# Jamol/kuma

Hardware: AMD Instinct MI355X
Metric: GiB/s device-resident WS frame mask/unmask, 64 KiB frames; % HBM peak (higher is better)
Workload: dtype u8

## Files before the change

### kuma_amd/csrc/kmws_common.hpp

```cpp
#pragma once
#include <hip/hip_runtime.h>
#include <stdint.h>
#include <string.h>

#include "kmws_gpu.h"

namespace kmws {

typedef uint32_t u32x4 __attribute__((ext_vector_type(4)));

constexpr int kBlock = 256;

struct WsHead {
    uint32_t status;
    uint32_t pad[3];
};
constexpr uint32_t kStatusBadDesc = 1u;
constexpr uint32_t kStatusBadHeader = 2u;
constexpr uint32_t kStatusLookbackTimeout = 4u;

__host__ __device__ __forceinline__ uint64_t splitmix64(uint64_t x)
{
    uint64_t z = x + 0x9E3779B97F4A7C15ull;
    z = (z ^ (z >> 30)) * 0xBF58476D1CE4E5B9ull;
    z = (z ^ (z >> 27)) * 0x94D049BB133111EBull;
    return z ^ (z >> 31);
}

__device__ __forceinline__ uint32_t rot_key(uint32_t key, uint64_t frame_off)
{
    return __builtin_rotateleft32(key, (uint32_t)(frame_off & 3u) * 8u);
}

__device__ __forceinline__ uint32_t dword_byte_mask(int lo, int hi, int d)
{
    int a = lo - 4 * d, b = hi - 4 * d;
    a = a < 0 ? 0 : a;
    b = b > 4 ? 4 : b;
    if (b <= a) return 0u;
    uint32_t hm = b >= 4 ? 0xFFFFFFFFu : ((1u << (8 * b)) - 1u);
    uint32_t lm = (1u << (8 * a)) - 1u;
    return hm & ~lm;
}

__device__ __forceinline__ uint64_t low_bytes64(int k)
{
    return k >= 8 ? ~0ull : ((1ull << (8 * k)) - 1ull);
}
__device__ __forceinline__ u32x4 word_byte_range(int lo, int hi)
{
    const int l0 = lo < 8 ? lo : 8, h0 = hi < 8 ? hi : 8;
    const int l1 = lo > 8 ? lo - 8 : 0, h1 = hi > 8 ? hi - 8 : 0;
    const uint64_t a = low_bytes64(h0) & ~low_bytes64(l0);
    const uint64_t b = low_bytes64(h1) & ~low_bytes64(l1);
    return u32x4{(uint32_t)a, (uint32_t)(a >> 32), (uint32_t)b, (uint32_t)(b >> 32)};
}

inline kmws_status hip_status(hipError_t e)
{
    return e == hipSuccess ? KMWS_OK : KMWS_ERR_FAILED;
}

kmws_status launch_zero(void* p, uint32_t bytes, hipStream_t s);

constexpr uint32_t kPieceWords = 4 * kBlock;
struct PieceRec {
    uint32_t frame;
    uint32_t piece;
};
inline uint64_t piece_count(uint64_t off, uint32_t len)
{
    if (len == 0) return 0;
    const uint64_t words = ((off + len + 15) >> 4) - (off >> 4);
    return (words + kPieceWords - 1) / kPieceWords;
}
kmws_status launch_unmask_pieces(uint8_t* base, const kmws_desc* descs, const PieceRec* pieces, uint32_t np,
                                 hipStream_t s);

int resolve_device(int device);
void note_device_batch(uint64_t bytes, hipStream_t stream);
bool device_batch_running(int device);

constexpr int kResMaxDescs = KMWS_RESIDENT_MAX_PAYLOADS;
constexpr uint64_t kResMaxBytes = KMWS_RESIDENT_MAX_BYTES;
constexpr uint64_t kResMaxBytesAsync = kResMaxBytes;
struct ResidentJob {
    int device = -1;
    int slot = -1;
    uint64_t seq = 0;
};
kmws_status resident_post(int device, const kmws_desc* descs, const uint8_t* dev_base, size_t n,
                          const kmws_desc* descs2, const uint8_t* dev_base2, size_t n2, ResidentJob* job,
                          uint64_t max_bytes = kResMaxBytes);
int resident_test(const ResidentJob& job);
kmws_status resident_wait(const ResidentJob& job);
kmws_status resident_unmask(int device, const kmws_desc* descs, const uint8_t* dev_base, size_t n,
                            const kmws_desc* descs2, const uint8_t* dev_base2, size_t n2);

}
```

### kuma_amd/csrc/kmws_unmask.hip

```cpp
#include "kmws_bench.h"
#include "kmws_common.hpp"
#include "kmws_frame_parse.hpp"

namespace kmws {

constexpr int kBufNT = 2;
constexpr int kBufferRsrcWord3 = 0x00020000;

__device__ __forceinline__ __amdgpu_buffer_rsrc_t tile_rsrc(uint8_t* base, uint64_t lo, uint64_t hi)
{
    return __builtin_amdgcn_make_buffer_rsrc(base + lo, (short)0, (int)((hi - lo + 15) & ~15ull), kBufferRsrcWord3);
}

template <bool NT>
__device__ __forceinline__ void store_word(const u32x4& val, __amdgpu_buffer_rsrc_t rs, uint32_t off)
{
    __builtin_amdgcn_raw_buffer_store_b128(val, rs, (int)off, 0, NT ? kBufNT : 0);
}

template <int V>
struct UnmaskCfg {
    static constexpr int kWords = kBlock * V;
    static constexpr uint64_t kTile = (uint64_t)kWords * 16u;
    static constexpr int kCap = kBlock;
};

__global__ void __launch_bounds__(kBlock) tile_map_kernel(const kmws_desc* __restrict__ d, uint32_t n,
                                                          uint64_t span, uint32_t tile_shift,
                                                          uint32_t* __restrict__ map,
                                                          WsHead* __restrict__ head)
{
    const uint32_t f = blockIdx.x * kBlock + threadIdx.x;
    if (f >= n) return;
    const kmws_desc df = d[f];
    const uint64_t next = (f + 1 < n) ? d[f + 1].off : span;
    if (df.off > span || df.off + (uint64_t)df.len > next) {
        atomicOr(&head->status, kStatusBadDesc);
        return;
    }
    const uint64_t start = f == 0 ? 0 : df.off;
    const uint64_t T = 1ull << tile_shift;
    const uint64_t b0 = (start + T - 1) >> tile_shift;
    const uint64_t b1 = (next + T - 1) >> tile_shift;
    for (uint64_t b = b0; b < b1; ++b) map[b] = f;
    if (f == n - 1) map[b1] = f;
}

__global__ void __launch_bounds__(kBlock) unpack_plan_kernel(const uint8_t* __restrict__ wire, uint64_t span,
                                                             const uint64_t* __restrict__ hdr_off, uint32_t n,
                                                             int mode, kmws_desc* __restrict__ out_desc,
                                                             uint16_t* __restrict__ out_flags,
                                                             uint8_t* __restrict__ out_err, uint32_t tile_shift,
                                                             uint32_t* __restrict__ map, WsHead* __restrict__ head)
{
    const uint32_t f = blockIdx.x * kBlock + threadIdx.x;
    if (f >= n) return;
    unpack_one(wire, span, hdr_off, n, f, mode, out_desc, out_flags, out_err, head);
    const uint64_t h = hdr_off[f];
    const uint64_t next = f + 1 < n ? hdr_off[f + 1] : span;
    if (h > next || next > span) {
        atomicOr(&head->status, kStatusBadDesc);
        return;
    }
    const uint64_t start = f == 0 ? 0 : h;
    const uint64_t T = 1ull << tile_shift;
    const uint64_t b0 = (start + T - 1) >> tile_shift;
    const uint64_t b1 = (next + T - 1) >> tile_shift;
    for (uint64_t b = b0; b < b1; ++b) map[b] = f;
    if (f == n - 1) map[b1] = f;
}

template <int V, bool FULL>
__device__ __forceinline__ void load_tile(const uint8_t* __restrict__ base, uint64_t tile_lo, uint64_t tile_hi,
                                          u32x4 (&v)[V])
{
    const int tid = threadIdx.x;
#pragma unroll
    for (int i = 0; i < V; ++i) {
        const uint64_t a = tile_lo + 16u * (uint64_t)(tid + kBlock * i);
        if (FULL || a < tile_hi) v[i] = __builtin_nontemporal_load(reinterpret_cast<const u32x4*>(base + a));
        else v[i] = u32x4{0, 0, 0, 0};
    }
}

template <int V, bool FULL, bool TWO = false, bool NT = true>
__device__ __forceinline__ void finish_tile(uint8_t* __restrict__ base, uint64_t tile_lo, uint64_t tile_hi,
                                            const kmws_desc* __restrict__ d, uint32_t n,
                                            const uint32_t* __restrict__ map, uint32_t tile, bool ok,
                                            const u32x4 (&v)[V], uint64_t* s_off, uint64_t* s_end, uint32_t* s_key,
                                            const u32x4* pre = nullptr)
{
    using Cfg = UnmaskCfg<V>;
    const int tid = threadIdx.x;
    const __amdgpu_buffer_rsrc_t rs = tile_rsrc(base, tile_lo, tile_hi);
    uint32_t f = map[tile];
    const uint32_t flast = map[tile + 1];

    const kmws_desc d0 = d[f < n ? f : 0];
    if (FULL && f < n && d0.off <= tile_lo && d0.off + d0.len >= tile_hi) {
        const uint32_t r = rot_key(d0.key, d0.off);
#pragma unroll
        for (int i = 0; i < V; ++i) {
            const uint64_t a = tile_lo + 16u * (uint64_t)(tid + kBlock * i);
            if (ok) store_word<NT>(v[i] ^ r, rs, (uint32_t)(a - tile_lo));
        }
        return;
    }

    if (TWO && FULL && flast <= f + 1 && f < n) {
        const kmws_desc d1 = flast > f && flast < n ? d[flast] : kmws_desc{~0ull, 0u, 0u};
        const uint32_t r0 = rot_key(d0.key, d0.off), r1 = rot_key(d1.key, d1.off);
        constexpr uint32_t T = (uint32_t)Cfg::kTile;
        auto rel = [&](uint64_t x) -> uint32_t {
            return x <= tile_lo ? 0u : (x - tile_lo >= T ? T : (uint32_t)(x - tile_lo));
        };
        const uint32_t s0 = rel(d0.off), t0 = rel(d0.off + d0.len);
        const uint32_t s1 = rel(d1.off), t1 = d1.len ? rel(d1.off + d1.len) : s1;
        u32x4 m[V];
#pragma unroll
        for (int i = 0; i < V; ++i) {
            const uint32_t x = 16u * (uint32_t)(tid + kBlock * i);
            u32x4 mm = u32x4{0, 0, 0, 0};
            if (s0 <= x && t0 >= x + 16) {
                mm = u32x4{r0, r0, r0, r0};
            } else if (s1 <= x && t1 >= x + 16) {
                mm = u32x4{r1, r1, r1, r1};
            } else {
                auto cl = [&](uint32_t y) -> int { return y <= x ? 0 : (y - x >= 16u ? 16 : (int)(y - x)); };
                mm = (word_byte_range(cl(s0), cl(t0)) & r0) | (word_byte_range(cl(s1), cl(t1)) & r1);
            }
            m[i] = mm;
        }
        __builtin_amdgcn_sched_barrier(0);
#pragma unroll
        for (int i = 0; i < V; ++i) {
            const uint64_t a = tile_lo + 16u * (uint64_t)(tid + kBlock * i);
            if (ok && (m[i].x | m[i].y | m[i].z | m[i].w) != 0u)
                store_word<NT>(v[i] ^ m[i], rs, (uint32_t)(a - tile_lo));
        }
        return;
    }

    u32x4 m[V];
#pragma unroll
    for (int i = 0; i < V; ++i) m[i] = u32x4{0, 0, 0, 0};
    auto round = [&](bool have, const u32x4& x) -> int {
        int valid = 0;
        if (have) {
            const uint64_t off = (uint64_t)x.x | ((uint64_t)x.y << 32);
            if (off < tile_hi) {
                valid = 1;
                s_off[tid] = off;
                s_end[tid] = off + x.z;
                s_key[tid] = x.w;
            }
        }
        const int cnt = __syncthreads_count(valid);
#pragma unroll
        for (int i = 0; i < V; ++i) {
            const uint64_t a = tile_lo + 16u * (uint64_t)(tid + kBlock * i);
            int lo = 0, hi = cnt;
            while (lo < hi) {
                const int mid = (lo + hi) >> 1;
                if (s_end[mid] <= a) lo = mid + 1; else hi = mid;
            }
            for (int j = lo; j < cnt; ++j) {
                const uint64_t o = s_off[j];
                if (o >= a + 16) break;
                const uint64_t e = s_end[j];
                const uint32_t r = rot_key(s_key[j], o);
                if (o <= a && e >= a + 16) {
                    m[i] |= u32x4{r, r, r, r};
                } else {
                    const int blo = o > a ? (int)(o - a) : 0;
                    const int bhi = e < a + 16 ? (int)(e - a) : 16;
                    m[i].x |= r & dword_byte_mask(blo, bhi, 0);
                    m[i].y |= r & dword_byte_mask(blo, bhi, 1);
                    m[i].z |= r & dword_byte_mask(blo, bhi, 2);
                    m[i].w |= r & dword_byte_mask(blo, bhi, 3);
                }
            }
        }
        __syncthreads();
        return cnt;
    };
    auto have_f = [&]() { return f + (uint32_t)tid < n && f + (uint32_t)tid <= flast; };
    auto load_f = [&]() { return have_f() ? *reinterpret_cast<const u32x4*>(d + f + tid) : u32x4{0, 0, 0, 0}; };
    int cnt = pre ? round(have_f(), *pre) : round(have_f(), load_f());
    while (cnt == Cfg::kCap) {
        f += Cfg::kCap;
        cnt = round(have_f(), load_f());
    }
#pragma unroll
    for (int i = 0; i < V; ++i) {
        const uint64_t a = tile_lo + 16u * (uint64_t)(tid + kBlock * i);
        const u32x4 mm = m[i];
        if (ok && (FULL || a < tile_hi) && (mm.x | mm.y | mm.z | mm.w) != 0u)
            store_word<NT>(v[i] ^ mm, rs, (uint32_t)(a - tile_lo));
    }
}

template <int V>
__global__ void __launch_bounds__(kBlock) unmask_tail_kernel(uint8_t* __restrict__ base, uint64_t span,
                                                             const kmws_desc* __restrict__ d, uint32_t n,
                                                             const uint32_t* __restrict__ map,
                                                             const WsHead* __restrict__ head, uint32_t tile)
{
    using Cfg = UnmaskCfg<V>;
    __shared__ uint64_t s_off[Cfg::kCap];
    __shared__ uint64_t s_end[Cfg::kCap];
    __shared__ uint32_t s_key[Cfg::kCap];
    const uint64_t tile_lo = (uint64_t)tile * Cfg::kTile;
    u32x4 v[V];
    load_tile<V, false>(base, tile_lo, span, v);
    __builtin_amdgcn_sched_barrier(0);
    finish_tile<V, false>(base, tile_lo, span, d, n, map, tile, (head->status & kStatusBadDesc) == 0, v, s_off, s_end, s_key);
}

template <int V, bool TWO = false, bool NT = true>
__global__ void __launch_bounds__(kBlock) unmask_split_kernel(uint8_t* __restrict__ base,
                                                              const kmws_desc* __restrict__ d, uint32_t n,
                                                              const uint32_t* __restrict__ map,
                                                              const WsHead* __restrict__ head, uint32_t nfull,
                                                              uint32_t k, uint32_t c, uint32_t b0, uint32_t w)
{
    using Cfg = UnmaskCfg<V>;
    __shared__ uint64_t s_off[Cfg::kCap];
    __shared__ uint64_t s_end[Cfg::kCap];
    __shared__ uint32_t s_key[Cfg::kCap];
    const uint32_t b = b0 + blockIdx.x;
    uint32_t tile = b;
    if (c == 0) {
        const uint32_t q = nfull / k;
        if (b < q * k) tile = (b % k) * q + b / k;
    } else if (w <= 1) {
        const uint64_t run = (uint64_t)k * c;
        if (b < nfull / run * run) {
            const uint32_t x = b % k, i = b / k;
            tile = (i / c) * (uint32_t)run + x * c + i % c;
        }
    } else {
        const uint32_t kg = k / w;
        const uint64_t run = (uint64_t)kg * c;
        const uint64_t per = (uint64_t)nfull / w / run * run;
        if (b < per * w) {
            const uint32_t x = b % k, i = b / k;
            const uint32_t g = x % w, xi = x / w;
            tile = (uint32_t)(g * per) + (i / c) * (uint32_t)run + xi * c + i % c;
        }
    }
    const uint64_t lo = (uint64_t)tile * Cfg::kTile;
    u32x4 v[V];
    if constexpr (!TWO) {
        const uint32_t f = map[tile], fl = map[tile + 1];
        const uint32_t fi = f + threadIdx.x;
        u32x4 pre = u32x4{0, 0, 0, 0};
        if (fi < n && fi <= fl) pre = *reinterpret_cast<const u32x4*>(d + fi);
        load_tile<V, true>(base, lo, lo + Cfg::kTile, v);
        __builtin_amdgcn_sched_barrier(0);
        finish_tile<V, true, TWO, NT>(base, lo, lo + Cfg::kTile, d, n, map, tile, (head->status & kStatusBadDesc) == 0, v, s_off, s_end,
                                      s_key, &pre);
        return;
    }
    load_tile<V, true>(base, lo, lo + Cfg::kTile, v);
    __builtin_amdgcn_sched_barrier(0);
    finish_tile<V, true, TWO, NT>(base, lo, lo + Cfg::kTile, d, n, map, tile, (head->status & kStatusBadDesc) == 0, v, s_off, s_end,
                                  s_key);
}

__global__ void __launch_bounds__(kBlock) unmask_pieces_kernel(uint8_t* __restrict__ base,
                                                               const kmws_desc* __restrict__ d,
                                                               const PieceRec* __restrict__ pieces)
{
    constexpr int V = kPieceWords / kBlock;
    const PieceRec pr = pieces[blockIdx.x];
    const kmws_desc x = d[pr.frame];
    const uint64_t end = x.off + x.len;
    const uint64_t w0 = (x.off >> 4) + (uint64_t)pr.piece * kPieceWords;
    const uint64_t wh = (end + 15) >> 4;
    const uint64_t w1 = wh < w0 + kPieceWords ? wh : w0 + kPieceWords;
    const uint32_t r = rot_key(x.key, x.off);
    u32x4 v[V];
#pragma unroll
    for (int i = 0; i < V; ++i) {
        const uint64_t w = w0 + threadIdx.x + (uint64_t)kBlock * i;
        v[i] = w < w1 ? *reinterpret_cast<const u32x4*>(base + 16 * w) : u32x4{0, 0, 0, 0};
    }
#pragma unroll
    for (int i = 0; i < V; ++i) {
        const uint64_t w = w0 + threadIdx.x + (uint64_t)kBlock * i;
        if (w >= w1) continue;
        const uint64_t a = 16 * w;
        if (a >= x.off && a + 16 <= end) {
            *reinterpret_cast<u32x4*>(base + a) = v[i] ^ r;
        } else {
            const uint64_t lo = a > x.off ? a : x.off, hi = a + 16 < end ? a + 16 : end;
            for (uint64_t q = lo; q < hi; ++q) {
                const uint32_t b = (uint32_t)(q - a);
                const uint32_t dw = (b & 8u) ? ((b & 4u) ? v[i].w : v[i].z) : ((b & 4u) ? v[i].y : v[i].x);
                base[q] = (uint8_t)((dw ^ r) >> (8 * (b & 3u)));
            }
        }
    }
}

__global__ void __launch_bounds__(kBlock) fill_synthetic_kernel(uint8_t* __restrict__ base, uint64_t bytes,
                                                                uint64_t seed)
{
    const uint64_t nw = bytes >> 4;
    const uint64_t stride = (uint64_t)gridDim.x * kBlock;
    for (uint64_t w = (uint64_t)blockIdx.x * kBlock + threadIdx.x; w < nw; w += stride) {
        const uint64_t a = splitmix64(seed + 2 * w), b = splitmix64(seed + 2 * w + 1);
        *reinterpret_cast<u32x4*>(base + 16 * w) =
            u32x4{(uint32_t)a, (uint32_t)(a >> 32), (uint32_t)b, (uint32_t)(b >> 32)};
    }
    if (blockIdx.x == 0 && threadIdx.x < (bytes & 15)) {
        const uint64_t i = (nw << 4) + threadIdx.x;
        base[i] = (uint8_t)(splitmix64(seed + (i >> 3)) >> (8 * (i & 7)));
    }
}

__global__ void __launch_bounds__(kBlock) uniform_descs_kernel(kmws_desc* __restrict__ d, uint32_t n,
                                                               uint64_t stride, uint32_t len, uint64_t key_seed)
{
    const uint32_t i = blockIdx.x * kBlock + threadIdx.x;
    if (i >= n) return;
    kmws_desc x;
    x.off = (uint64_t)i * stride;
    x.len = len;
    x.key = (uint32_t)splitmix64(key_seed + i);
    d[i] = x;
}

constexpr int kCheckBytes = 4096;

__global__ void __launch_bounds__(kBlock) check_unmasked_kernel(const uint8_t* __restrict__ base, uint64_t bytes,
                                                                uint64_t seed, const kmws_desc* __restrict__ d,
                                                                uint32_t n, unsigned long long* mismatches)
{
    __shared__ uint32_t s_first;
    const uint64_t nblk = (bytes + kCheckBytes - 1) / kCheckBytes;
    unsigned long long bad = 0;
    for (uint64_t blk = blockIdx.x; blk < nblk; blk += gridDim.x) {
    const uint64_t blk_lo = blk * kCheckBytes;
    __syncthreads();
    if (threadIdx.x == 0) {
        uint32_t lo = 0, hi = n;
        while (lo < hi) {
            const uint32_t mid = (lo + hi) >> 1;
            if (d[mid].off + d[mid].len <= blk_lo) lo = mid + 1; else hi = mid;
        }
        s_first = lo;
    }
    __syncthreads();
    uint32_t f = s_first;
    const uint64_t p0 = blk_lo + 16u * threadIdx.x;
    for (int k = 0; k < 16; ++k) {
        const uint64_t p = p0 + k;
        if (p >= bytes) break;
        while (f < n && d[f].off + d[f].len <= p) ++f;
        uint8_t expect = (uint8_t)(splitmix64(seed + (p >> 3)) >> (8 * (p & 7)));
        if (f < n && d[f].off <= p) {
            const uint32_t key = d[f].key;
            expect ^= (uint8_t)(key >> (8 * ((p - d[f].off) & 3)));
        }
        bad += base[p] != expect;
    }
    }
    if (bad) atomicAdd(mismatches, bad);
}

constexpr int kUnmaskV = 4;
using ProdCfg = UnmaskCfg<kUnmaskV>;

constexpr unsigned kUnmaskBlocksPerCu = 2;
constexpr uint32_t kUnmaskStaticLds = ProdCfg::kCap * (8 + 8 + 4);

static unsigned unmask_lds_pad_device()
{
    static thread_local int dev_cached = -1;
    static thread_local unsigned pad = 0;
    int dev = 0;
    if (hipGetDevice(&dev) != hipSuccess) return 0;
    if (dev != dev_cached) {
        int lds = 0;
        pad = 0;
        if (
            hipDeviceGetAttribute(&lds, hipDeviceAttributeMaxSharedMemoryPerMultiprocessor, dev) == hipSuccess &&
            lds > 0) {
            const unsigned per_block = (unsigned)lds / (kUnmaskBlocksPerCu + 1) + 1;
            pad = per_block > kUnmaskStaticLds ? per_block - kUnmaskStaticLds : 0u;
        }
        dev_cached = dev;
    }
    return pad;
}

static unsigned unmask_lds_pad(uint64_t span, uint32_t n)
{
    return n && span / n >= ProdCfg::kTile ? unmask_lds_pad_device() : 0u;
}

static uint32_t ilog2_u64(uint64_t x)
{
    uint32_t r = 0;
    while ((1ull << r) < x) ++r;
    return r;
}

static kmws_status check_ws(uint64_t span, size_t ws_bytes, uint64_t* ntiles_out)
{
    const uint64_t ntiles = (span + ProdCfg::kTile - 1) / ProdCfg::kTile;
    if (ntiles > 0x7FFFFFFFull) return KMWS_ERR_INVALID_PARAM;
    if (ws_bytes < sizeof(WsHead) + (ntiles + 1) * sizeof(uint32_t)) return KMWS_ERR_BUFFER_TOO_SMALL;
    *ntiles_out = ntiles;
    return KMWS_OK;
}

static kmws_status launch_plan(uint64_t span, const kmws_desc* descs, uint32_t n, void* workspace, size_t ws_bytes,
                               hipStream_t s)
{
    uint64_t ntiles = 0;
    kmws_status st = check_ws(span, ws_bytes, &ntiles);
    if (st != KMWS_OK) return st;
    WsHead* head = static_cast<WsHead*>(workspace);
    if (launch_zero(head, sizeof(WsHead), s) != KMWS_OK) return KMWS_ERR_FAILED;
    if (n == 0 || span == 0) return KMWS_OK;
    hipLaunchKernelGGL(tile_map_kernel, dim3((n + kBlock - 1) / kBlock), dim3(kBlock), 0, s, descs, n, span,
                       ilog2_u64(ProdCfg::kTile), reinterpret_cast<uint32_t*>(head + 1), head);
    return hip_status(hipGetLastError());
}

struct Split {
    uint32_t k, c, w;
};
constexpr uint32_t kKindMask = 0xFFu;
constexpr uint32_t kSchedTemporal = KMWS_SCHED_TEMPORAL_STORES;
constexpr uint32_t kSchedNT = KMWS_SCHED_NT_STORES;
static uint32_t default_schedule(uint64_t span, uint32_t n)
{
    return n && span / n >= ProdCfg::kTile ? KMWS_SCHED_SPLIT4 : KMWS_SCHED_GROUPED_RUNS;
}

static bool split_of(uint32_t kind, Split* sp)
{
    switch (kind) {
    case KMWS_SCHED_GROUPED_RUNS: *sp = {8u, 16u, 2u}; return true;
    case KMWS_SCHED_IN_ORDER: *sp = {1u, 0u, 1u}; return true;
    case KMWS_SCHED_SPLIT2: *sp = {2u, 0u, 1u}; return true;
    case KMWS_SCHED_SPLIT8: *sp = {8u, 0u, 1u}; return true;
    case KMWS_SCHED_XCD_RUNS: *sp = {8u, 16u, 1u}; return true;
    case KMWS_SCHED_SPLIT4: *sp = {4u, 0u, 1u}; return true;
    default: return false;
    }
}

static bool valid_schedule(uint32_t code)
{
    Split sp;
    const uint32_t store = code & (kSchedTemporal | kSchedNT);
    return split_of(code & kKindMask, &sp) && store != (kSchedTemporal | kSchedNT) &&
           (code & ~(kKindMask | kSchedTemporal | kSchedNT)) == 0;
}

static bool temporal_stores(uint32_t code) { return (code & kSchedTemporal) != 0; }

static kmws_status launch_apply(uint32_t code, uint8_t* base, uint64_t span, const kmws_desc* descs, uint32_t n,
                                const void* workspace, size_t ws_bytes, hipStream_t s)
{
    Split sp;
    if (!valid_schedule(code) || !split_of(code & kKindMask, &sp)) return KMWS_ERR_INVALID_PARAM;
    uint64_t ntiles = 0;
    kmws_status st = check_ws(span, ws_bytes, &ntiles);
    if (st != KMWS_OK) return st;
    if (n == 0 || span == 0) return KMWS_OK;
    const WsHead* head = static_cast<const WsHead*>(workspace);
    const uint32_t* map = reinterpret_cast<const uint32_t*>(head + 1);
    const uint64_t nfull = span / ProdCfg::kTile;
    const bool temporal = temporal_stores(code);
    constexpr uint64_t kMaxBlocks = (1ull << 32) / kBlock / 2;
    const unsigned lds_pad = unmask_lds_pad(span, n);
    for (uint64_t b0 = 0; b0 < nfull; b0 += kMaxBlocks) {
        const dim3 grid((uint32_t)(nfull - b0 < kMaxBlocks ? nfull - b0 : kMaxBlocks));
        const uint32_t nf = (uint32_t)nfull, bb = (uint32_t)b0;
        if (lds_pad && !temporal)
            hipLaunchKernelGGL((unmask_split_kernel<kUnmaskV, true, true>), grid, dim3(kBlock), lds_pad, s, base, descs,
                               n, map, head, nf, sp.k, sp.c, bb, sp.w);
        else if (lds_pad)
            hipLaunchKernelGGL((unmask_split_kernel<kUnmaskV, true, false>), grid, dim3(kBlock), lds_pad, s, base,
                               descs, n, map, head, nf, sp.k, sp.c, bb, sp.w);
        else if (!temporal)
            hipLaunchKernelGGL((unmask_split_kernel<kUnmaskV, false, true>), grid, dim3(kBlock), 0, s, base, descs, n,
                               map, head, nf, sp.k, sp.c, bb, sp.w);
        else
            hipLaunchKernelGGL((unmask_split_kernel<kUnmaskV, false, false>), grid, dim3(kBlock), 0, s, base, descs,
                               n, map, head, nf, sp.k, sp.c, bb, sp.w);
    }
    if (ntiles > nfull)
        hipLaunchKernelGGL(unmask_tail_kernel<kUnmaskV>, dim3(1), dim3(kBlock), 0, s, base, span, descs, n, map, head,
                           (uint32_t)nfull);
    return hip_status(hipGetLastError());
}

static bool bad_args(const uint8_t* base, const kmws_desc* descs, uint32_t n, const void* ws)
{
    return !ws || (n && (!base || !descs)) || (reinterpret_cast<uintptr_t>(base) & 15u);
}

__global__ void __launch_bounds__(64) zero_kernel(uint64_t* __restrict__ p, uint32_t words)
{
    for (uint32_t i = threadIdx.x; i < words; i += 64) p[i] = 0;
}

kmws_status launch_zero(void* p, uint32_t bytes, hipStream_t s)
{
    if (!p || (bytes & 7u) || bytes > 4096) return KMWS_ERR_INVALID_PARAM;
    hipLaunchKernelGGL(zero_kernel, dim3(1), dim3(64), 0, s, static_cast<uint64_t*>(p), bytes / 8);
    return hip_status(hipGetLastError());
}

kmws_status launch_unmask_pieces(uint8_t* base, const kmws_desc* descs, const PieceRec* pieces, uint32_t np,
                                 hipStream_t s)
{
    if (np == 0) return KMWS_OK;
    if (!base || !descs || !pieces) return KMWS_ERR_INVALID_PARAM;
    hipLaunchKernelGGL(unmask_pieces_kernel, dim3(np), dim3(kBlock), 0, s, base, descs, pieces);
    return hip_status(hipGetLastError());
}
}

using namespace kmws;

extern "C" {

size_t kmws_unmask_workspace_size(uint64_t span)
{
    const uint64_t ntiles = (span + ProdCfg::kTile - 1) / ProdCfg::kTile;
    return sizeof(WsHead) + (size_t)(ntiles + 1) * sizeof(uint32_t);
}

kmws_status kmws_unmask_batch(uint8_t* base, uint64_t span, const kmws_desc* descs, uint32_t n,
                              void* workspace, size_t workspace_bytes, void* stream)
{
    if (bad_args(base, descs, n, workspace)) return KMWS_ERR_INVALID_PARAM;
    kmws_status st = launch_plan(span, descs, n, workspace, workspace_bytes, static_cast<hipStream_t>(stream));
    if (st != KMWS_OK) return st;
    return kmws_unmask_apply(base, span, descs, n, workspace, workspace_bytes, stream);
}

kmws_status kmws_unmask_plan(uint64_t span, const kmws_desc* descs, uint32_t n, void* workspace,
                             size_t workspace_bytes, void* stream)
{
    if (!workspace || (n && !descs)) return KMWS_ERR_INVALID_PARAM;
    return launch_plan(span, descs, n, workspace, workspace_bytes, static_cast<hipStream_t>(stream));
}

kmws_status kmws_unmask_apply(uint8_t* base, uint64_t span, const kmws_desc* descs, uint32_t n,
                              const void* workspace, size_t workspace_bytes, void* stream)
{
    return kmws_unmask_apply_sched(base, span, descs, n, workspace, workspace_bytes, -1, stream);
}

kmws_status kmws_unmask_apply_sched(uint8_t* base, uint64_t span, const kmws_desc* descs, uint32_t n,
                                    const void* workspace, size_t workspace_bytes, int schedule, void* stream)
{
    if (bad_args(base, descs, n, workspace)) return KMWS_ERR_INVALID_PARAM;
    const uint32_t code = schedule < 0 ? default_schedule(span, n) : (uint32_t)schedule;
    kmws::note_device_batch(2 * span, static_cast<hipStream_t>(stream));
    return launch_apply(code, base, span, descs, n, workspace, workspace_bytes, static_cast<hipStream_t>(stream));
}

int kmws_unmask_default_schedule(uint64_t span, uint32_t n) { return (int)default_schedule(span, n); }

kmws_status kmws_unpack_unmask(uint8_t* wire, uint64_t wire_len, const uint64_t* hdr_off, uint32_t n, int mode,
                               kmws_desc* out_desc, uint16_t* out_flags, uint8_t* out_err, void* workspace,
                               size_t workspace_bytes, int schedule, void* stream)
{
    if (bad_args(wire, out_desc, n, workspace) || (n && !hdr_off) ||
        (mode != KMWS_MODE_CLIENT && mode != KMWS_MODE_SERVER))
        return KMWS_ERR_INVALID_PARAM;
    const uint32_t code = schedule < 0 ? default_schedule(wire_len, n) : (uint32_t)schedule;
    if (!valid_schedule(code)) return KMWS_ERR_INVALID_PARAM;
    uint64_t ntiles = 0;
    kmws_status st = check_ws(wire_len, workspace_bytes, &ntiles);
    if (st != KMWS_OK) return st;
    hipStream_t s = static_cast<hipStream_t>(stream);
    WsHead* head = static_cast<WsHead*>(workspace);
    if (launch_zero(head, sizeof(WsHead), s) != KMWS_OK) return KMWS_ERR_FAILED;
    if (n == 0) return KMWS_OK;
    kmws::note_device_batch(2 * wire_len, s);
    hipLaunchKernelGGL(unpack_plan_kernel, dim3((n + kBlock - 1) / kBlock), dim3(kBlock), 0, s, wire, wire_len, hdr_off,
                       n, mode, out_desc, out_flags, out_err, ilog2_u64(ProdCfg::kTile),
                       reinterpret_cast<uint32_t*>(head + 1), head);
    st = hip_status(hipGetLastError());
    if (st != KMWS_OK) return st;
    return launch_apply(code, wire, wire_len, out_desc, n, workspace, workspace_bytes, s);
}

int kmws_unmask_autotune(uint8_t* base, uint64_t span, const kmws_desc* descs, uint32_t n, void* workspace,
                         size_t workspace_bytes, void* stream)
{
    if (bad_args(base, descs, n, workspace)) return KMWS_ERR_INVALID_PARAM;
    hipStream_t s = static_cast<hipStream_t>(stream);
    kmws_status st = launch_plan(span, descs, n, workspace, workspace_bytes, s);
    if (st != KMWS_OK) return st;
    static const uint32_t kinds[] = {KMWS_SCHED_GROUPED_RUNS, KMWS_SCHED_SPLIT4, KMWS_SCHED_SPLIT8,
                                     KMWS_SCHED_XCD_RUNS,     KMWS_SCHED_SPLIT2, KMWS_SCHED_IN_ORDER};
    hipEvent_t e0, e1;
    if (hipEventCreate(&e0) != hipSuccess) return KMWS_ERR_FAILED;
    if (hipEventCreate(&e1) != hipSuccess) {
        (void)hipEventDestroy(e0);
        return KMWS_ERR_FAILED;
    }
    float best = 1e30f;
    uint32_t pick = default_schedule(span, n);
    for (int rep = 0; rep < 2 && st == KMWS_OK; ++rep) {
        for (uint32_t kind : kinds) {
            for (uint32_t store : {kSchedNT, kSchedTemporal}) {
                const uint32_t g = kind | store;
                if (hipEventRecord(e0, s) != hipSuccess) { st = KMWS_ERR_FAILED; break; }
                for (int k = 0; k < 2 && st == KMWS_OK; ++k)
                    st = launch_apply(g, base, span, descs, n, workspace, workspace_bytes, s);
                if (st != KMWS_OK || hipEventRecord(e1, s) != hipSuccess || hipEventSynchronize(e1) != hipSuccess) {
                    st = st != KMWS_OK ? st : KMWS_ERR_FAILED;
                    break;
                }
                float ms = 0;
                (void)hipEventElapsedTime(&ms, e0, e1);
                if (rep == 1 && ms < best) {
                    best = ms;
                    pick = g;
                }
            }
            if (st != KMWS_OK) break;
        }
    }
    (void)hipEventDestroy(e0);
    (void)hipEventDestroy(e1);
    if (st != KMWS_OK) return st;
    return (int)pick;
}

kmws_status kmws_read_status(const void* workspace, uint32_t* status_out, void* stream)
{
    if (!workspace || !status_out) return KMWS_ERR_INVALID_PARAM;
    hipStream_t s = static_cast<hipStream_t>(stream);
    hipError_t e = hipMemcpyAsync(status_out, workspace, sizeof(uint32_t), hipMemcpyDeviceToHost, s);
    if (e == hipSuccess) e = hipStreamSynchronize(s);
    return hip_status(e);
}

int kmws_device_count(void)
{
    int n = 0;
    if (hipGetDeviceCount(&n) != hipSuccess) return 0;
    int good = 0;
    for (int i = 0; i < n; ++i) {
        hipDeviceProp_t p;
        if (hipGetDeviceProperties(&p, i) == hipSuccess && strncmp(p.gcnArchName, "gfx950", 6) == 0) ++good;
    }
    return good;
}


void* kmws_arena_alloc(uint64_t bytes, int device, int* contiguous)
{
    if (contiguous) *contiguous = 0;
    if (bytes == 0) return nullptr;
    int prev = -1;
    if (hipGetDevice(&prev) != hipSuccess) return nullptr;
    if (device != prev && hipSetDevice(device) != hipSuccess) return nullptr;
    void* p = nullptr;
    if (hipExtMallocWithFlags(&p, bytes, hipDeviceMallocContiguous) == hipSuccess && p) {
        if (contiguous) *contiguous = 1;
    } else {
        (void)hipGetLastError();
        p = nullptr;
        if (hipMalloc(&p, bytes) != hipSuccess) {
            (void)hipGetLastError();
            p = nullptr;
        }
    }
    if (device != prev) (void)hipSetDevice(prev);
    return p;
}

void kmws_arena_free(void* p, int device)
{
    if (!p) return;
    int prev = -1;
    if (hipGetDevice(&prev) != hipSuccess) return;
    if (device != prev) (void)hipSetDevice(device);
    (void)hipFree(p);
    if (device != prev) (void)hipSetDevice(prev);
}

int64_t kmws_arena_place(uint8_t* arena, uint64_t arena_bytes, uint64_t span, uint64_t step, void* stream,
                         float* frac_out, uint32_t max_out)
{
    constexpr uint64_t kFrame = 65536;
    if (!arena || span == 0 || span > arena_bytes || step == 0 || (step & 15u) ||
        (reinterpret_cast<uintptr_t>(arena) & 15u) || span / kFrame > 0xFFFFFFFFull)
        return KMWS_ERR_INVALID_PARAM;
    hipStream_t s = static_cast<hipStream_t>(stream);
    const uint32_t n = (uint32_t)((span + kFrame - 1) / kFrame);
    const size_t ws_bytes = kmws_unmask_workspace_size(span);
    kmws_desc* d = nullptr;
    void* ws = nullptr;
    hipEvent_t e0 = nullptr, e1 = nullptr;
    int64_t result = KMWS_ERR_FAILED;
    if (hipMalloc(reinterpret_cast<void**>(&d), (size_t)n * sizeof(kmws_desc)) != hipSuccess ||
        hipMalloc(&ws, ws_bytes) != hipSuccess || hipEventCreate(&e0) != hipSuccess ||
        hipEventCreate(&e1) != hipSuccess) {
        (void)hipGetLastError();
    } else {
        hipLaunchKernelGGL(uniform_descs_kernel, dim3((n + kBlock - 1) / kBlock), dim3(kBlock), 0, s, d, n, kFrame,
                           (uint32_t)kFrame, 0x706c6163ull);
        const uint32_t last_len = (uint32_t)(span - (uint64_t)(n - 1) * kFrame);
        kmws_status st = hip_status(hipMemcpyAsync(&d[n - 1].len, &last_len, sizeof(last_len),
                                                   hipMemcpyHostToDevice, s));
        if (st == KMWS_OK) st = hip_status(hipStreamSynchronize(s));
        float best = 1e30f;
        uint64_t pick = 0;
        uint32_t k = 0;
        for (uint64_t off = 0; st == KMWS_OK && off + span <= arena_bytes; off += step, ++k) {
            float t = 1e30f;
            for (int rep = 0; rep < 4 && st == KMWS_OK; ++rep) {
                st = launch_plan(span, d, n, ws, ws_bytes, s);
                if (st == KMWS_OK) st = hip_status(hipEventRecord(e0, s));
                const uint32_t g = (rep & 1 ? KMWS_SCHED_SPLIT8 : KMWS_SCHED_SPLIT4) | kSchedNT;
                for (int i = 0; i < 2 && st == KMWS_OK; ++i)
                    st = launch_apply(g, arena + off, span, d, n, ws, ws_bytes, s);
                if (st == KMWS_OK) st = hip_status(hipEventRecord(e1, s));
                if (st == KMWS_OK) st = hip_status(hipEventSynchronize(e1));
                float ms = 0;
                if (st == KMWS_OK && hipEventElapsedTime(&ms, e0, e1) == hipSuccess && ms < t) t = ms;
            }
            if (st != KMWS_OK) break;
            if (frac_out && k < max_out) frac_out[k] = (float)(2.0 * (2.0 * span + 16.0 * n) / (t * 1e-3) / 8e12);
            if (t < best) {
                best = t;
                pick = off;
            }
        }
        uint32_t status = 0;
        if (st == KMWS_OK) st = hip_status(hipMemcpy(&status, ws, sizeof(status), hipMemcpyDeviceToHost));
        result = st != KMWS_OK ? (int64_t)st : (status != 0 ? (int64_t)KMWS_ERR_FAILED : (int64_t)pick);
    }
    if (e0) (void)hipEventDestroy(e0);
    if (e1) (void)hipEventDestroy(e1);
    if (ws) (void)hipFree(ws);
    if (d) (void)hipFree(d);
    return result;
}

kmws_status kmws_fill_synthetic(uint8_t* base, uint64_t bytes, uint64_t seed, void* stream)
{
    if (!base && bytes) return KMWS_ERR_INVALID_PARAM;
    if ((reinterpret_cast<uintptr_t>(base) & 15u)) return KMWS_ERR_INVALID_PARAM;
    if (bytes == 0) return KMWS_OK;
    hipLaunchKernelGGL(fill_synthetic_kernel, dim3(8192), dim3(kBlock), 0, static_cast<hipStream_t>(stream), base,
                       bytes, seed);
    return hip_status(hipGetLastError());
}

kmws_status kmws_fill_uniform_descs(kmws_desc* descs, uint32_t n, uint64_t stride, uint32_t len,
                                    uint64_t key_seed, void* stream)
{
    if (!descs && n) return KMWS_ERR_INVALID_PARAM;
    if (n == 0) return KMWS_OK;
    hipLaunchKernelGGL(uniform_descs_kernel, dim3((n + kBlock - 1) / kBlock), dim3(kBlock), 0,
                       static_cast<hipStream_t>(stream), descs, n, stride, len, key_seed);
    return hip_status(hipGetLastError());
}

kmws_status kmws_check_unmasked(const uint8_t* base, uint64_t bytes, uint64_t seed, const kmws_desc* descs,
                                uint32_t n, unsigned long long* mismatches, void* stream)
{
    if ((!base && bytes) || !mismatches) return KMWS_ERR_INVALID_PARAM;
    if (bytes == 0) return KMWS_OK;
    uint64_t nb = (bytes + kCheckBytes - 1) / kCheckBytes;
    if (nb > 65536) nb = 65536;
    hipLaunchKernelGGL(check_unmasked_kernel, dim3((uint32_t)nb), dim3(kBlock), 0, static_cast<hipStream_t>(stream),
                       base, bytes, seed, descs, n, mismatches);
    return hip_status(hipGetLastError());
}

}
```

Before: 3064.

## Precompute per-tile covered flag and rotated key in tile map records

The tile map now stores an 8-byte record per tile: the frame index with a 'fully covered' flag bit, plus the pre-rotated mask key. The unmask kernel loads both adjacent records in one read and takes the XOR fast path without a dependent descriptor load. Other changes in the same commit: tile loads go through buffer-load intrinsics, the large-tile path's stores use a non-temporal cache policy with an extra SC1 bit, and the block-to-tile mapping is precomputed on the host with shifts instead of divisions. Compile-time-gated phase timestamp diagnostics are also added. The map doubles in workspace size, and the flag trick only works while the frame count stays below 2^31.

```diff
diff --git a/kuma_amd/csrc/kmws_common.hpp b/kuma_amd/csrc/kmws_common.hpp
--- a/kuma_amd/csrc/kmws_common.hpp
+++ b/kuma_amd/csrc/kmws_common.hpp
@@ -56,6 +56,84 @@
     return u32x4{(uint32_t)a, (uint32_t)(a >> 32), (uint32_t)b, (uint32_t)(b >> 32)};
 }
 
+struct alignas(8) TileRec {
+    uint32_t frame;
+    uint32_t rkey;
+};
+struct alignas(8) TileRecPair {
+    TileRec at, next;
+};
+constexpr uint32_t kTileRecCovered = 0x80000000u;
+constexpr uint32_t kTileRecMaxFlagged = 0x80000000u;
+__host__ __device__ __forceinline__ bool tile_rec_covered(TileRec r, uint32_t n)
+{
+    return n < kTileRecMaxFlagged && (r.frame & kTileRecCovered) != 0u;
+}
+__host__ __device__ __forceinline__ uint32_t tile_rec_frame(TileRec r, uint32_t n)
+{
+    return n < kTileRecMaxFlagged ? r.frame & ~kTileRecCovered : r.frame;
+}
+
+struct Split {
+    uint32_t k, c, w;
+};
+struct TileMapping {
+    uint32_t whole;
+    uint32_t part;
+    uint32_t lk;
+    uint32_t lc;
+    uint32_t lw;
+    uint32_t runs;
+};
+__host__ __device__ __forceinline__ uint32_t ilog2_pow2(uint32_t x)
+{
+    uint32_t r = 0;
+    while ((1u << r) < x) ++r;
+    return r;
+}
+__host__ __device__ __forceinline__ TileMapping tile_mapping(uint32_t nfull, Split sp)
+{
+    TileMapping m;
+    m.lk = ilog2_pow2(sp.k);
+    m.lw = ilog2_pow2(sp.w);
+    m.runs = sp.c != 0u;
+    if (!m.runs) {
+        m.lc = 0;
+        m.part = nfull >> m.lk;
+        m.whole = m.part << m.lk;
+    } else {
+        m.lc = ilog2_pow2(sp.c);
+        const uint32_t lrun = m.lk - m.lw + m.lc;
+        m.part = ((nfull >> m.lw) >> lrun) << lrun;
+        m.whole = m.part << m.lw;
+    }
+    return m;
+}
+__host__ __device__ __forceinline__ uint32_t tile_of_block(uint32_t b, TileMapping m)
+{
+    if (b >= m.whole) return b;
+    const uint32_t x = b & ((1u << m.lk) - 1u), i = b >> m.lk;
+    if (!m.runs) return x * m.part + i;
+    const uint32_t g = x & ((1u << m.lw) - 1u), xi = x >> m.lw;
+    return g * m.part + ((i >> m.lc) << (m.lk - m.lw + m.lc)) + (xi << m.lc) + (i & ((1u << m.lc) - 1u));
+}
+__host__ __device__ __forceinline__ uint32_t tile_of_block(uint32_t b, uint32_t nfull, Split sp)
+{
+    return tile_of_block(b, tile_mapping(nfull, sp));
+}
+__host__ __device__ __forceinline__ bool split_of(uint32_t kind, Split* sp)
+{
+    switch (kind) {
+    case KMWS_SCHED_GROUPED_RUNS: *sp = {8u, 16u, 2u}; return true;
+    case KMWS_SCHED_IN_ORDER: *sp = {1u, 0u, 1u}; return true;
+    case KMWS_SCHED_SPLIT2: *sp = {2u, 0u, 1u}; return true;
+    case KMWS_SCHED_SPLIT8: *sp = {8u, 0u, 1u}; return true;
+    case KMWS_SCHED_XCD_RUNS: *sp = {8u, 16u, 1u}; return true;
+    case KMWS_SCHED_SPLIT4: *sp = {4u, 0u, 1u}; return true;
+    default: return false;
+    }
+}
+
 inline kmws_status hip_status(hipError_t e)
 {
     return e == hipSuccess ? KMWS_OK : KMWS_ERR_FAILED;
diff --git a/kuma_amd/csrc/kmws_unmask.hip b/kuma_amd/csrc/kmws_unmask.hip
--- a/kuma_amd/csrc/kmws_unmask.hip
+++ b/kuma_amd/csrc/kmws_unmask.hip
@@ -4,7 +4,10 @@
 
 namespace kmws {
 
-constexpr int kBufNT = 2;
+constexpr int kPolPlain = 0, kPolNT = 2, kPolNTSC1 = 18;
+constexpr int kPolStreamStoreLarge = kPolNTSC1;
+constexpr int kPolStreamStoreSmall = kPolNT;
+constexpr int kPolStreamLoad = kPolNT;
 constexpr int kBufferRsrcWord3 = 0x00020000;
 
 __device__ __forceinline__ __amdgpu_buffer_rsrc_t tile_rsrc(uint8_t* base, uint64_t lo, uint64_t hi)
@@ -12,11 +15,36 @@
     return __builtin_amdgcn_make_buffer_rsrc(base + lo, (short)0, (int)((hi - lo + 15) & ~15ull), kBufferRsrcWord3);
 }
 
-template <bool NT>
+template <int POL>
 __device__ __forceinline__ void store_word(const u32x4& val, __amdgpu_buffer_rsrc_t rs, uint32_t off)
 {
-    __builtin_amdgcn_raw_buffer_store_b128(val, rs, (int)off, 0, NT ? kBufNT : 0);
-}
+    __builtin_amdgcn_raw_buffer_store_b128(val, rs, (int)off, 0, POL);
+}
+
+#ifdef KMWS_DIAG_PHASE_STAMPS
+constexpr int kDiagStamps = 6;
+constexpr uint32_t kDiagEvery = 1024;
+__device__ uint64_t* g_diag_stamps = nullptr;
+__device__ uint32_t g_diag_slots = 0;
+#define KMWS_STAMP(st, i)                              \
+    do {                                               \
+        __builtin_amdgcn_sched_barrier(0);             \
+        if (st) (st)[i] = __builtin_amdgcn_s_memtime(); \
+        __builtin_amdgcn_sched_barrier(0);             \
+    } while (0)
+#define KMWS_STAMP_AFTER(st, i, waitcnt)               \
+    do {                                               \
+        __builtin_amdgcn_sched_barrier(0);             \
+        if (st) {                                      \
+            asm volatile("s_waitcnt " waitcnt ::: "memory"); \
+            (st)[i] = __builtin_amdgcn_s_memtime();    \
+        }                                              \
+        __builtin_amdgcn_sched_barrier(0);             \
+    } while (0)
+#else
+#define KMWS_STAMP(st, i) do { (void)(st); } while (0)
+#define KMWS_STAMP_AFTER(st, i, waitcnt) do { (void)(st); } while (0)
+#endif
 
 template <int V>
 struct UnmaskCfg {
@@ -25,9 +53,24 @@
     static constexpr int kCap = kBlock;
 };
 
+__device__ __forceinline__ void write_tile_recs(TileRec* __restrict__ map, uint32_t f, uint32_t n, uint64_t off,
+                                                uint32_t len, uint32_t key, uint64_t b0, uint64_t b1,
+                                                uint32_t tile_shift)
+{
+    const uint64_t end = off + len;
+    const uint32_t r = rot_key(key, off);
+    const bool flagged = n < kTileRecMaxFlagged;
+    for (uint64_t b = b0; b < b1; ++b) {
+        const uint64_t lo = b << tile_shift, hi = (b + 1) << tile_shift;
+        const bool cov = flagged && off <= lo && end >= hi;
+        map[b] = TileRec{cov ? f | kTileRecCovered : f, cov ? r : 0u};
+    }
+    if (f == n - 1) map[b1] = TileRec{f, 0u};
+}
+
 __global__ void __launch_bounds__(kBlock) tile_map_kernel(const kmws_desc* __restrict__ d, uint32_t n,
                                                           uint64_t span, uint32_t tile_shift,
-                                                          uint32_t* __restrict__ map,
+                                                          TileRec* __restrict__ map,
                                                           WsHead* __restrict__ head)
 {
     const uint32_t f = blockIdx.x * kBlock + threadIdx.x;
@@ -42,8 +85,7 @@
     const uint64_t T = 1ull << tile_shift;
     const uint64_t b0 = (start + T - 1) >> tile_shift;
     const uint64_t b1 = (next + T - 1) >> tile_shift;
-    for (uint64_t b = b0; b < b1; ++b) map[b] = f;
-    if (f == n - 1) map[b1] = f;
+    write_tile_recs(map, f, n, df.off, df.len, df.key, b0, b1, tile_shift);
 }
 
 __global__ void __launch_bounds__(kBlock) unpack_plan_kernel(const uint8_t* __restrict__ wire, uint64_t span,
@@ -51,11 +93,11 @@
                                                              int mode, kmws_desc* __restrict__ out_desc,
                                                              uint16_t* __restrict__ out_flags,
                                                              uint8_t* __restrict__ out_err, uint32_t tile_shift,
-                                                             uint32_t* __restrict__ map, WsHead* __restrict__ head)
+                                                             TileRec* __restrict__ map, WsHead* __restrict__ head)
 {
     const uint32_t f = blockIdx.x * kBlock + threadIdx.x;
     if (f >= n) return;
-    unpack_one(wire, span, hdr_off, n, f, mode, out_desc, out_flags, out_err, head);
+    const kmws_desc df = unpack_one(wire, span, hdr_off, n, f, mode, out_desc, out_flags, out_err, head);
     const uint64_t h = hdr_off[f];
     const uint64_t next = f + 1 < n ? hdr_off[f + 1] : span;
     if (h > next || next > span) {
@@ -66,46 +108,51 @@
     const uint64_t T = 1ull << tile_shift;
     const uint64_t b0 = (start + T - 1) >> tile_shift;
     const uint64_t b1 = (next + T - 1) >> tile_shift;
-    for (uint64_t b = b0; b < b1; ++b) map[b] = f;
-    if (f == n - 1) map[b1] = f;
-}
-
-template <int V, bool FULL>
-__device__ __forceinline__ void load_tile(const uint8_t* __restrict__ base, uint64_t tile_lo, uint64_t tile_hi,
+    write_tile_recs(map, f, n, df.off, df.len, df.key, b0, b1, tile_shift);
+}
+
+template <int V, bool FULL, int POL = kPolStreamLoad>
+__device__ __forceinline__ void load_tile(uint8_t* __restrict__ base, uint64_t tile_lo, uint64_t tile_hi,
                                           u32x4 (&v)[V])
 {
     const int tid = threadIdx.x;
+    const __amdgpu_buffer_rsrc_t rs = tile_rsrc(base, tile_lo, tile_hi);
 #pragma unroll
     for (int i = 0; i < V; ++i) {
-        const uint64_t a = tile_lo + 16u * (uint64_t)(tid + kBlock * i);
-        if (FULL || a < tile_hi) v[i] = __builtin_nontemporal_load(reinterpret_cast<const u32x4*>(base + a));
+        const uint32_t x = 16u * (uint32_t)(tid + kBlock * i);
+        if (FULL || tile_lo + x < tile_hi) v[i] = __builtin_amdgcn_raw_buffer_load_b128(rs, (int)x, 0, POL);
         else v[i] = u32x4{0, 0, 0, 0};
     }
 }
 
 template <int V, bool FULL, bool TWO = false, bool NT = true>
 __device__ __forceinline__ void finish_tile(uint8_t* __restrict__ base, uint64_t tile_lo, uint64_t tile_hi,
-                                            const kmws_desc* __restrict__ d, uint32_t n,
-                                            const uint32_t* __restrict__ map, uint32_t tile, bool ok,
-                                            const u32x4 (&v)[V], uint64_t* s_off, uint64_t* s_end, uint32_t* s_key,
-                                            const u32x4* pre = nullptr)
+                                            const kmws_desc* __restrict__ d, uint32_t n, TileRec rec,
+                                            TileRec rec_next, bool ok, const u32x4 (&v)[V], uint64_t* s_off,
+                                            uint64_t* s_end, uint32_t* s_key, const u32x4* pre = nullptr,
+                                            uint64_t* stamps = nullptr)
 {
     using Cfg = UnmaskCfg<V>;
+    constexpr int SP = !NT ? kPolPlain : (TWO ? kPolStreamStoreLarge : kPolStreamStoreSmall);
     const int tid = threadIdx.x;
     const __amdgpu_buffer_rsrc_t rs = tile_rsrc(base, tile_lo, tile_hi);
-    uint32_t f = map[tile];
-    const uint32_t flast = map[tile + 1];
-
-    const kmws_desc d0 = d[f < n ? f : 0];
-    if (FULL && f < n && d0.off <= tile_lo && d0.off + d0.len >= tile_hi) {
-        const uint32_t r = rot_key(d0.key, d0.off);
+    KMWS_STAMP_AFTER(stamps, 3, "lgkmcnt(0)");
+
+    if (FULL && tile_rec_covered(rec, n)) {
+        const uint32_t r = rec.rkey;
+        KMWS_STAMP_AFTER(stamps, 4, "vmcnt(3)");
 #pragma unroll
         for (int i = 0; i < V; ++i) {
             const uint64_t a = tile_lo + 16u * (uint64_t)(tid + kBlock * i);
-            if (ok) store_word<NT>(v[i] ^ r, rs, (uint32_t)(a - tile_lo));
-        }
+            if (ok) store_word<SP>(v[i] ^ r, rs, (uint32_t)(a - tile_lo));
+        }
+        KMWS_STAMP(stamps, 5);
         return;
     }
+
+    uint32_t f = tile_rec_frame(rec, n);
+    const uint32_t flast = tile_rec_frame(rec_next, n);
+    const kmws_desc d0 = d[f < n ? f : 0];
 
     if (TWO && FULL && flast <= f + 1 && f < n) {
         const kmws_desc d1 = flast > f && flast < n ? d[flast] : kmws_desc{~0ull, 0u, 0u};
@@ -136,7 +183,7 @@
         for (int i = 0; i < V; ++i) {
             const uint64_t a = tile_lo + 16u * (uint64_t)(tid + kBlock * i);
             if (ok && (m[i].x | m[i].y | m[i].z | m[i].w) != 0u)
-                store_word<NT>(v[i] ^ m[i], rs, (uint32_t)(a - tile_lo));
+                store_word<SP>(v[i] ^ m[i], rs, (uint32_t)(a - tile_lo));
         }
         return;
     }
@@ -196,14 +243,14 @@
         const uint64_t a = tile_lo + 16u * (uint64_t)(tid + kBlock * i);
         const u32x4 mm = m[i];
         if (ok && (FULL || a < tile_hi) && (mm.x | mm.y | mm.z | mm.w) != 0u)
-            store_word<NT>(v[i] ^ mm, rs, (uint32_t)(a - tile_lo));
+            store_word<SP>(v[i] ^ mm, rs, (uint32_t)(a - tile_lo));
     }
 }
 
 template <int V>
 __global__ void __launch_bounds__(kBlock) unmask_tail_kernel(uint8_t* __restrict__ base, uint64_t span,
                                                              const kmws_desc* __restrict__ d, uint32_t n,
-                                                             const uint32_t* __restrict__ map,
+                                                             const TileRec* __restrict__ map,
                                                              const WsHead* __restrict__ head, uint32_t tile)
 {
     using Cfg = UnmaskCfg<V>;
@@ -214,58 +261,56 @@
     u32x4 v[V];
     load_tile<V, false>(base, tile_lo, span, v);
     __builtin_amdgcn_sched_barrier(0);
-    finish_tile<V, false>(base, tile_lo, span, d, n, map, tile, (head->status & kStatusBadDesc) == 0, v, s_off, s_end, s_key);
+    finish_tile<V, false>(base, tile_lo, span, d, n, map[tile], map[tile + 1], (head->status & kStatusBadDesc) == 0,
+                          v, s_off, s_end, s_key);
 }
 
 template <int V, bool TWO = false, bool NT = true>
 __global__ void __launch_bounds__(kBlock) unmask_split_kernel(uint8_t* __restrict__ base,
                                                               const kmws_desc* __restrict__ d, uint32_t n,
-                                                              const uint32_t* __restrict__ map,
-                                                              const WsHead* __restrict__ head, uint32_t nfull,
-                                                              uint32_t k, uint32_t c, uint32_t b0, uint32_t w)
+                                                              const TileRec* __restrict__ map,
+                                                              const WsHead* __restrict__ head, TileMapping tm,
+                                                              uint32_t b0)
 {
     using Cfg = UnmaskCfg<V>;
     __shared__ uint64_t s_off[Cfg::kCap];
     __shared__ uint64_t s_end[Cfg::kCap];
     __shared__ uint32_t s_key[Cfg::kCap];
-    const uint32_t b = b0 + blockIdx.x;
-    uint32_t tile = b;
-    if (c == 0) {
-        const uint32_t q = nfull / k;
-        if (b < q * k) tile = (b % k) * q + b / k;
-    } else if (w <= 1) {
-        const uint64_t run = (uint64_t)k * c;
-        if (b < nfull / run * run) {
-            const uint32_t x = b % k, i = b / k;
-            tile = (i / c) * (uint32_t)run + x * c + i % c;
-        }
-    } else {
-        const uint32_t kg = k / w;
-        const uint64_t run = (uint64_t)kg * c;
-        const uint64_t per = (uint64_t)nfull / w / run * run;
-        if (b < per * w) {
-            const uint32_t x = b % k, i = b / k;
-            const uint32_t g = x % w, xi = x / w;
-            tile = (uint32_t)(g * per) + (i / c) * (uint32_t)run + xi * c + i % c;
-        }
-    }
+#ifdef KMWS_DIAG_PHASE_STAMPS
+    uint64_t st[kDiagStamps] = {};
+#else
+    uint64_t* const st = nullptr;
+#endif
+    KMWS_STAMP(st, 0);
+    const uint32_t tile = tile_of_block(b0 + blockIdx.x, tm);
     const uint64_t lo = (uint64_t)tile * Cfg::kTile;
+    const TileRecPair recs = *reinterpret_cast<const TileRecPair*>(map + tile);
+    const TileRec rec = recs.at, rec_next = recs.next;
+    const uint32_t status = head->status;
     u32x4 v[V];
     if constexpr (!TWO) {
-        const uint32_t f = map[tile], fl = map[tile + 1];
+        const uint32_t f = tile_rec_frame(rec, n), fl = tile_rec_frame(rec_next, n);
         const uint32_t fi = f + threadIdx.x;
         u32x4 pre = u32x4{0, 0, 0, 0};
         if (fi < n && fi <= fl) pre = *reinterpret_cast<const u32x4*>(d + fi);
         load_tile<V, true>(base, lo, lo + Cfg::kTile, v);
         __builtin_amdgcn_sched_barrier(0);
-        finish_tile<V, true, TWO, NT>(base, lo, lo + Cfg::kTile, d, n, map, tile, (head->status & kStatusBadDesc) == 0, v, s_off, s_end,
-                                      s_key, &pre);
+        finish_tile<V, true, TWO, NT>(base, lo, lo + Cfg::kTile, d, n, rec, rec_next,
+                                      (status & kStatusBadDesc) == 0, v, s_off, s_end, s_key, &pre);
         return;
     }
+    __builtin_amdgcn_sched_barrier(0);
+    KMWS_STAMP(st, 1);
     load_tile<V, true>(base, lo, lo + Cfg::kTile, v);
     __builtin_amdgcn_sched_barrier(0);
-    finish_tile<V, true, TWO, NT>(base, lo, lo + Cfg::kTile, d, n, map, tile, (head->status & kStatusBadDesc) == 0, v, s_off, s_end,
-                                  s_key);
+    KMWS_STAMP(st, 2);
+    finish_tile<V, true, TWO, NT>(base, lo, lo + Cfg::kTile, d, n, rec, rec_next, (status & kStatusBadDesc) == 0, v,
+                                  s_off, s_end, s_key, nullptr, st);
+#ifdef KMWS_DIAG_PHASE_STAMPS
+    const uint32_t blk = b0 + blockIdx.x;
+    if (blk % kDiagEvery == 0 && blk / kDiagEvery < g_diag_slots && threadIdx.x == 0 && st[5] != 0)
+        for (int i = 0; i < kDiagStamps; ++i) g_diag_stamps[(uint64_t)(blk / kDiagEvery) * kDiagStamps + i] = st[i];
+#endif
 }
 
 __global__ void __launch_bounds__(kBlock) unmask_pieces_kernel(uint8_t* __restrict__ base,
@@ -412,7 +457,7 @@
 {
     const uint64_t ntiles = (span + ProdCfg::kTile - 1) / ProdCfg::kTile;
     if (ntiles > 0x7FFFFFFFull) return KMWS_ERR_INVALID_PARAM;
-    if (ws_bytes < sizeof(WsHead) + (ntiles + 1) * sizeof(uint32_t)) return KMWS_ERR_BUFFER_TOO_SMALL;
+    if (ws_bytes < sizeof(WsHead) + (ntiles + 1) * sizeof(TileRec)) return KMWS_ERR_BUFFER_TOO_SMALL;
     *ntiles_out = ntiles;
     return KMWS_OK;
 }
@@ -427,32 +472,16 @@
     if (launch_zero(head, sizeof(WsHead), s) != KMWS_OK) return KMWS_ERR_FAILED;
     if (n == 0 || span == 0) return KMWS_OK;
     hipLaunchKernelGGL(tile_map_kernel, dim3((n + kBlock - 1) / kBlock), dim3(kBlock), 0, s, descs, n, span,
-                       ilog2_u64(ProdCfg::kTile), reinterpret_cast<uint32_t*>(head + 1), head);
+                       ilog2_u64(ProdCfg::kTile), reinterpret_cast<TileRec*>(head + 1), head);
     return hip_status(hipGetLastError());
 }
 
-struct Split {
-    uint32_t k, c, w;
-};
 constexpr uint32_t kKindMask = 0xFFu;
 constexpr uint32_t kSchedTemporal = KMWS_SCHED_TEMPORAL_STORES;
 constexpr uint32_t kSchedNT = KMWS_SCHED_NT_STORES;
 static uint32_t default_schedule(uint64_t span, uint32_t n)
 {
     return n && span / n >= ProdCfg::kTile ? KMWS_SCHED_SPLIT4 : KMWS_SCHED_GROUPED_RUNS;
-}
-
-static bool split_of(uint32_t kind, Split* sp)
-{
-    switch (kind) {
-    case KMWS_SCHED_GROUPED_RUNS: *sp = {8u, 16u, 2u}; return true;
-    case KMWS_SCHED_IN_ORDER: *sp = {1u, 0u, 1u}; return true;
-    case KMWS_SCHED_SPLIT2: *sp = {2u, 0u, 1u}; return true;
-    case KMWS_SCHED_SPLIT8: *sp = {8u, 0u, 1u}; return true;
-    case KMWS_SCHED_XCD_RUNS: *sp = {8u, 16u, 1u}; return true;
-    case KMWS_SCHED_SPLIT4: *sp = {4u, 0u, 1u}; return true;
-    default: return false;
-    }
 }
 
 static bool valid_schedule(uint32_t code)
@@ -475,26 +504,27 @@
     if (st != KMWS_OK) return st;
     if (n == 0 || span == 0) return KMWS_OK;
     const WsHead* head = static_cast<const WsHead*>(workspace);
-    const uint32_t* map = reinterpret_cast<const uint32_t*>(head + 1);
+    const TileRec* map = reinterpret_cast<const TileRec*>(head + 1);
     const uint64_t nfull = span / ProdCfg::kTile;
     const bool temporal = temporal_stores(code);
     constexpr uint64_t kMaxBlocks = (1ull << 32) / kBlock / 2;
     const unsigned lds_pad = unmask_lds_pad(span, n);
+    const TileMapping tm = tile_mapping((uint32_t)nfull, sp);
     for (uint64_t b0 = 0; b0 < nfull; b0 += kMaxBlocks) {
         const dim3 grid((uint32_t)(nfull - b0 < kMaxBlocks ? nfull - b0 : kMaxBlocks));
-        const uint32_t nf = (uint32_t)nfull, bb = (uint32_t)b0;
+        const uint32_t bb = (uint32_t)b0;
         if (lds_pad && !temporal)
             hipLaunchKernelGGL((unmask_split_kernel<kUnmaskV, true, true>), grid, dim3(kBlock), lds_pad, s, base, descs,
-                               n, map, head, nf, sp.k, sp.c, bb, sp.w);
+                               n, map, head, tm, bb);
         else if (lds_pad)
             hipLaunchKernelGGL((unmask_split_kernel<kUnmaskV, true, false>), grid, dim3(kBlock), lds_pad, s, base,
-                               descs, n, map, head, nf, sp.k, sp.c, bb, sp.w);
+                               descs, n, map, head, tm, bb);
         else if (!temporal)
             hipLaunchKernelGGL((unmask_split_kernel<kUnmaskV, false, true>), grid, dim3(kBlock), 0, s, base, descs, n,
-                               map, head, nf, sp.k, sp.c, bb, sp.w);
+                               map, head, tm, bb);
         else
             hipLaunchKernelGGL((unmask_split_kernel<kUnmaskV, false, false>), grid, dim3(kBlock), 0, s, base, descs,
-                               n, map, head, nf, sp.k, sp.c, bb, sp.w);
+                               n, map, head, tm, bb);
     }
     if (ntiles > nfull)
         hipLaunchKernelGGL(unmask_tail_kernel<kUnmaskV>, dim3(1), dim3(kBlock), 0, s, base, span, descs, n, map, head,
@@ -536,7 +566,7 @@
 size_t kmws_unmask_workspace_size(uint64_t span)
 {
     const uint64_t ntiles = (span + ProdCfg::kTile - 1) / ProdCfg::kTile;
-    return sizeof(WsHead) + (size_t)(ntiles + 1) * sizeof(uint32_t);
+    return sizeof(WsHead) + (size_t)(ntiles + 1) * sizeof(TileRec);
 }
 
 kmws_status kmws_unmask_batch(uint8_t* base, uint64_t span, const kmws_desc* descs, uint32_t n,
@@ -591,7 +621,7 @@
     kmws::note_device_batch(2 * wire_len, s);
     hipLaunchKernelGGL(unpack_plan_kernel, dim3((n + kBlock - 1) / kBlock), dim3(kBlock), 0, s, wire, wire_len, hdr_off,
                        n, mode, out_desc, out_flags, out_err, ilog2_u64(ProdCfg::kTile),
-                       reinterpret_cast<uint32_t*>(head + 1), head);
+                       reinterpret_cast<TileRec*>(head + 1), head);
     st = hip_status(hipGetLastError());
     if (st != KMWS_OK) return st;
     return launch_apply(code, wire, wire_len, out_desc, n, workspace, workspace_bytes, s);
@@ -649,6 +679,17 @@
     if (e == hipSuccess) e = hipStreamSynchronize(s);
     return hip_status(e);
 }
+
+#ifdef KMWS_DIAG_PHASE_STAMPS
+kmws_status kmws_diag_set_stamps(uint64_t* buf, uint32_t slots)
+{
+    const uint32_t s = buf ? slots : 0u;
+    if (hipMemcpyToSymbol(HIP_SYMBOL(g_diag_slots), &s, sizeof(s)) != hipSuccess ||
+        hipMemcpyToSymbol(HIP_SYMBOL(g_diag_stamps), &buf, sizeof(buf)) != hipSuccess)
+        return KMWS_ERR_FAILED;
+    return hip_status(hipDeviceSynchronize());
+}
+#endif
 
 int kmws_device_count(void)
 {
```

After: 3095, median of 6. 1.01x the previous value.
